# raahii/dcvgan

Measured on AMD Instinct MI355X. Metric: videos/sec per G+D step, 16x64x64 RGB+depth, higher is better.
Workload: dtype f32

## Files before the change

dcvgan_amd/csrc/conv_mfma.hip:

```cpp
#include "dcv_common.h"

#include <algorithm>
#include <cstdlib>
#include <map>
#include <mutex>
#include <string>
#include <type_traits>
#include <vector>

namespace dcv {

thread_local char g_err[512] = {0};
std::atomic<uint64_t> g_launches{0};
thread_local char g_last_kernel[160] = {0};
#define DCV_NOTE_KERNEL(...) snprintf(g_last_kernel, sizeof(g_last_kernel), __VA_ARGS__)

typedef float f32x16 __attribute__((ext_vector_type(16)));
typedef __bf16 bf16x8 __attribute__((ext_vector_type(8)));

std::atomic<int> g_precision{0};
struct BnView {
    const float* bx; const float* gamma; const float* beta; const float* mean; const float* invstd;
    int64_t bx_sn;
    int32_t bx_sc, bx_sh, cbn, act;
    float slope;
};

__device__ __forceinline__ bf16x8 pack_bf16x8(const float (&t)[8]) {
    typedef float f32x2_ __attribute__((ext_vector_type(2)));
    typedef __bf16 bf16x2_ __attribute__((ext_vector_type(2)));
    typedef uint32_t u32x4_ __attribute__((ext_vector_type(4)));
    u32x4_ w;
#pragma unroll
    for (int q = 0; q < 4; ++q) {
        const f32x2_ f = {t[2 * q], t[2 * q + 1]};
        w[q] = __builtin_bit_cast(uint32_t, __builtin_convertvector(f, bf16x2_));
    }
    return __builtin_bit_cast(bf16x8, w);
}

__device__ __forceinline__ void split3_bf16x8(const float (&t)[8], bf16x8 (&o)[3]) {
    typedef float f32x2_ __attribute__((ext_vector_type(2)));
    typedef __bf16 bf16x2_ __attribute__((ext_vector_type(2)));
    typedef uint32_t u32x4_ __attribute__((ext_vector_type(4)));
    u32x4_ h, m, l;
#pragma unroll
    for (int q = 0; q < 4; ++q) {
        const f32x2_ f = {t[2 * q], t[2 * q + 1]};
        const uint32_t hw = __builtin_bit_cast(uint32_t, __builtin_convertvector(f, bf16x2_));
        const f32x2_ r = {f[0] - __builtin_bit_cast(float, hw << 16), f[1] - __builtin_bit_cast(float, hw & 0xffff0000u)};
        const uint32_t mw = __builtin_bit_cast(uint32_t, __builtin_convertvector(r, bf16x2_));
        const f32x2_ r2 = {r[0] - __builtin_bit_cast(float, mw << 16), r[1] - __builtin_bit_cast(float, mw & 0xffff0000u)};
        h[q] = hw; m[q] = mw; l[q] = __builtin_bit_cast(uint32_t, __builtin_convertvector(r2, bf16x2_));
    }
    o[0] = __builtin_bit_cast(bf16x8, h); o[1] = __builtin_bit_cast(bf16x8, m); o[2] = __builtin_bit_cast(bf16x8, l);
}
#ifdef DCV_X6_NO_PHASES
#define X6_PHASE(IT) false
#else
#define X6_PHASE(IT) ((((IT) >> 3) & 1) != 0)
#endif
#define DCV_MFMA_X6(ACC, A3, B3)                                                              \
    {                                                                                         \
        ACC = __builtin_amdgcn_mfma_f32_32x32x16_bf16((A3)[2], (B3)[0], ACC, 0, 0, 0);        \
        ACC = __builtin_amdgcn_mfma_f32_32x32x16_bf16((A3)[0], (B3)[2], ACC, 0, 0, 0);        \
        ACC = __builtin_amdgcn_mfma_f32_32x32x16_bf16((A3)[1], (B3)[1], ACC, 0, 0, 0);        \
        ACC = __builtin_amdgcn_mfma_f32_32x32x16_bf16((A3)[1], (B3)[0], ACC, 0, 0, 0);        \
        ACC = __builtin_amdgcn_mfma_f32_32x32x16_bf16((A3)[0], (B3)[1], ACC, 0, 0, 0);        \
        ACC = __builtin_amdgcn_mfma_f32_32x32x16_bf16((A3)[0], (B3)[0], ACC, 0, 0, 0);        \
    }

#ifdef DCV_STAMP
__device__ unsigned long long g_stamp[4096][4][6];
#define STAMP(var) unsigned long long var = clock64(); __builtin_amdgcn_sched_barrier(0)
#else
#define STAMP(var) __builtin_amdgcn_sched_barrier(0)
#endif

struct KEntry {
    int32_t x_off;
    uint32_t tapsel;
    int32_t w_off;
    int32_t pad;
};

struct DimTaps {
    int32_t n;
    int32_t mul, base;
    int32_t size;
    int32_t delta[8];
};

struct GatherArgs {
    const float* x;
    float* y;
    const float* wp;
    const int32_t* koff;
    const uint32_t* ksel;
    int32_t M, OC, OCp, KIT;
    FastDiv div_sp, div_hw, div_w;
    int32_t OD, OH, OW, pad0;
    DimTaps td, th, tw;
    int64_t x_sn;
    int32_t x_sd, x_sh, x_sw, x_back;
    int64_t y_sn, y_sc, y_sd, y_sh, y_sw, y_off;
    int32_t act, accumulate;
    float slope, pad2;
    float* slab;
    int32_t kper, Mp;
    int32_t structured, s_log2p, s_stepA, s_stepD;
    int32_t s_local[16];
    uint32_t s_sel[16];
    int32_t patch, p_G, p_log2nh, p_log2tr;
    int32_t p_log2ow, p_iwp, p_ihmin, p_iwmin4;
    int32_t p_dw1, p_sc4, slab_mp, p_pad2;
    FastDiv p_gpr;
    float* stat;
    int32_t stat_ntm, stat_cls;
    const float* gate;
    float gate_slope;
    int32_t rag_m0;
};

struct GatherArgsPack {
    GatherArgs c[4];
};

__device__ __forceinline__ float apply_act(float v, int act, float slope) {
    if (act == DCV_ACT_LEAKY) return v > 0.f ? v : v * slope;
    if (act == DCV_ACT_TANH) return tanhf(v);
    return v;
}

__device__ __forceinline__ uint32_t dim_mask(const DimTaps t, int o, int shift) {
    uint32_t m = 0;
    const int p0 = o * t.mul + t.base;
#pragma unroll
    for (int u = 0; u < 8; ++u) {
        const int p = p0 + t.delta[u];
        m |= ((unsigned)p < (unsigned)t.size && u < t.n) ? (1u << (shift + u)) : 0u;
    }
    return m;
}


template <int TOC, int TM, int ACT, bool GENERIC>
__device__ __forceinline__ void store_tiles(const f32x16 (&acc)[TOC][TM], const __amdgpu_buffer_rsrc_t yrs, const uint32_t (&voff)[TM],
                                            const int ocw, const int lhi, const int OC, const uint32_t y_sc4, const int act, const float slope,
                                            const bool accumulate, const __amdgpu_buffer_rsrc_t grs, const bool gated, const float gslope) {
#pragma unroll
    for (int j = 0; j < TM; ++j)
#pragma unroll
        for (int i = 0; i < TOC; ++i)
#pragma unroll
            for (int r = 0; r < 16; ++r) {
                const int ocr = i * 32 + (r & 3) + 8 * (r >> 2);
                const uint32_t soff = (uint32_t)(ocw + ocr) * y_sc4;
                float v = acc[i][j][r];
                uint32_t vo = voff[j];
                if constexpr (GENERIC) {
                    if (ocw + ocr + 4 * lhi >= OC) vo = 0x80000000u;
                    if (accumulate) v += __builtin_bit_cast(float, __builtin_amdgcn_raw_buffer_load_b32(yrs, vo, soff, 0));
                    if (gated) v *= __builtin_bit_cast(float, __builtin_amdgcn_raw_buffer_load_b32(grs, vo, soff, 0)) > 0.f ? 1.f : gslope;
                    v = apply_act(v, act, slope);
                } else {
                    if constexpr (ACT == DCV_ACT_LEAKY) v = v > 0.f ? v : v * slope;
                    if constexpr (ACT == DCV_ACT_TANH) v = tanhf(v);
                }
                __builtin_amdgcn_raw_buffer_store_b32(__builtin_bit_cast(uint32_t, v), yrs, vo, soff, 0);
            }
}

__device__ __forceinline__ uint32_t out_voffset(const GatherArgs& a, int m, uint32_t n0, int lhi, uint32_t y_sc4) {
    if (m >= a.M) return 0x80000000u;
    const uint32_t n = fdiv((uint32_t)m, a.div_sp);
    uint32_t r0 = (uint32_t)m - n * a.div_sp.div;
    const uint32_t od = fdiv(r0, a.div_hw);
    r0 -= od * a.div_hw.div;
    const uint32_t oh = fdiv(r0, a.div_w);
    const uint32_t ow = r0 - oh * a.div_w.div;
    return 4u * (uint32_t)((int)(n - n0) * (int)a.y_sn + (int)od * (int)a.y_sd + (int)oh * (int)a.y_sh + (int)ow * (int)a.y_sw) + (uint32_t)(4 * lhi) * y_sc4;
}

template <int TOC, int TM>
__device__ __forceinline__ void gather_epilogue(const GatherArgs& a, const f32x16 (&acc)[TOC][TM], int m0, int mcol0, int l31, int lhi, int ocw, uint32_t n0) {
    const int OC = a.OC, OCp = a.OCp, act = a.act;
    const bool accumulate = a.accumulate != 0;
    const float slope = a.slope;
    const uint32_t y_sc4 = (uint32_t)a.y_sc * 4u;
    const __amdgpu_buffer_rsrc_t yrs = __builtin_amdgcn_make_buffer_rsrc(a.y + a.y_off + (int64_t)n0 * a.y_sn, 0, a.p_pad2 == 0x5701 ? 0u : 0x80000000u, 0x00020000);
    uint32_t voff[TM];
#pragma unroll
    for (int j = 0; j < TM; ++j) voff[j] = out_voffset(a, m0 + mcol0 + j * 32 + l31, n0, lhi, y_sc4);
    const bool gated = a.gate != nullptr;
    const __amdgpu_buffer_rsrc_t grs = __builtin_amdgcn_make_buffer_rsrc(const_cast<float*>(gated ? a.gate : a.y) + a.y_off + (int64_t)n0 * a.y_sn, 0, 0x80000000u, 0x00020000);
    if (OC == OCp && !accumulate && !gated) {
        if (act == DCV_ACT_NONE) store_tiles<TOC, TM, DCV_ACT_NONE, false>(acc, yrs, voff, ocw, lhi, OC, y_sc4, act, slope, false, grs, false, 0.f);
        else if (act == DCV_ACT_LEAKY) store_tiles<TOC, TM, DCV_ACT_LEAKY, false>(acc, yrs, voff, ocw, lhi, OC, y_sc4, act, slope, false, grs, false, 0.f);
        else store_tiles<TOC, TM, DCV_ACT_TANH, false>(acc, yrs, voff, ocw, lhi, OC, y_sc4, act, slope, false, grs, false, 0.f);
    } else {
        store_tiles<TOC, TM, 0, true>(acc, yrs, voff, ocw, lhi, OC, y_sc4, act, slope, accumulate, grs, gated, a.gate_slope);
    }
}

template <int TOC, int TM, int WOC, int WM, bool STRUCT>
__global__ __launch_bounds__(256, 3) void gather_gemm_kernel(const GatherArgs a) {
    constexpr int BN = 32 * TOC * WOC;
    constexpr int BM = 32 * TM * WM;
    constexpr int XPT = 16 * BM / 256;
    static_assert(WOC * WM == 4, "4 waves");
    static_assert(BM == 64 || BM == 128 || BM == 256, "BM");
    constexpr int WF4 = 16 * BN / 4;
    constexpr int WPT = (WF4 + 255) / 256;

    __shared__ __attribute__((aligned(16))) float Xs[2][16][BM];
    __shared__ __attribute__((aligned(16))) float Ws[2][16][BN];

    const int tid = threadIdx.x;
    const int lane = tid & 63;
    const int wave = __builtin_amdgcn_readfirstlane(tid >> 6);
    const int woc = wave / WM, wm = wave % WM;

    const int tiles_oc = a.OCp / BN;
    const int oc_t = blockIdx.x % tiles_oc;
    const int m_t = blockIdx.x / tiles_oc;
    const int oc0 = oc_t * BN;
    const int m0 = m_t * BM;

    const uint32_t n0 = fdiv((uint32_t)m0, a.div_sp);
    const __amdgpu_buffer_rsrc_t xrs = __builtin_amdgcn_make_buffer_rsrc(
        const_cast<float*>(a.x + (int64_t)n0 * a.x_sn), 0, 0x80000000u, 0x00020000);

    const int lm = tid % BM;
    const int ksub = __builtin_amdgcn_readfirstlane(tid / BM);
    int xbase4 = 0;
    uint32_t vmask = 0;
    {
        const int m = m0 + lm;
        if (m < a.M) {
            const uint32_t n = fdiv((uint32_t)m, a.div_sp);
            uint32_t r = (uint32_t)m - n * a.div_sp.div;
            const uint32_t od = fdiv(r, a.div_hw);
            r -= od * a.div_hw.div;
            const uint32_t oh = fdiv(r, a.div_w);
            const uint32_t ow = r - oh * a.div_w.div;
            vmask = dim_mask(a.td, (int)od, 0) | dim_mask(a.th, (int)oh, 8) | dim_mask(a.tw, (int)ow, 16);
            xbase4 = 4 * ((int)((int64_t)(n - n0) * a.x_sn) + ((int)od * a.td.mul + a.td.base) * a.x_sd +
                          ((int)oh * a.th.mul + a.th.base) * a.x_sh + ((int)ow * a.tw.mul + a.tw.base) * a.x_sw);
        }
    }

    f32x16 acc[TOC][TM];
#pragma unroll
    for (int i = 0; i < TOC; ++i)
#pragma unroll
        for (int j = 0; j < TM; ++j)
#pragma unroll
            for (int r = 0; r < 16; ++r) acc[i][j][r] = 0.f;

    float xv[XPT];
    float4 wv[WPT];

    uint32_t vloc[STRUCT ? XPT : 1];
    if constexpr (STRUCT) {
#pragma unroll
        for (int i = 0; i < XPT; ++i) {
            const int r = ksub * XPT + i;
            const uint32_t sel = a.s_sel[r];
            vloc[i] = ((vmask & sel) == sel) ? (uint32_t)(xbase4 + a.s_local[r]) : 0x80000000u;
        }
    }

    auto load_tile = [&](int it) {
        if constexpr (STRUCT) {
// ... 419 lines not shown
        if constexpr (DSTEP)
            while (nx < nst && !DCV_STEP_LIVE(DCV_IT(nx))) ++nx;
        STAMP(q0);
        asm volatile("s_waitcnt vmcnt(0)" ::: "memory");
        __syncthreads();
        STAMP(q1);
        __builtin_amdgcn_s_setprio(2);
        const int itn = DCV_IT(nx < nst ? nx : j);
        const int soffn = (itn >> a.s_log2p) * a.s_stepA + (itn & ((1 << a.s_log2p) - 1)) * a.s_stepD;
        j = nx;
        DCV_ISSUE_W(itn, buf ^ 1)
        const float* xt = Xs + buf * 16 * BM;
        const float* wt = Ws + buf * WSZ;
        if constexpr (BF == 2) {
#pragma unroll
            for (int i = 0; i < (PATCH ? NS : XPT); ++i) DCV_ISSUE_X(itn, soffn, buf ^ 1, i)
            bf16x8 a8[TOC][3], b8[TM][3];
#pragma unroll
            for (int i = 0; i < TOC; ++i)
#pragma unroll
                for (int pc = 0; pc < 3; ++pc)
                    a8[i][pc] = *reinterpret_cast<const bf16x8*>(reinterpret_cast<const char*>(wt) + 16 * ((pc * 2 + lhi) * BN + (woc * TOC + i) * 32 + l31));
            float tb[TM][8];
#pragma unroll
            for (int jj = 0; jj < TM; ++jj)
#pragma unroll
                for (int q = 0; q < 8; ++q)
                    tb[jj][q] = PATCH ? *reinterpret_cast<const float*>(reinterpret_cast<const char*>(xt) + (fbb[PATCH ? jj : 0] + koff8[PATCH ? q : 0]))
                                      : xt[(8 * lhi + q) * BM + (wm * TM + jj) * 32 + l31];
            split3_bf16x8(tb[0], b8[0]);
            if (X6_PHASE(it_cur) != x6_neg) {
                x6_neg = !x6_neg;
#pragma unroll
                for (int i = 0; i < TOC; ++i)
#pragma unroll
                    for (int jj = 0; jj < TM; ++jj)
#pragma unroll
                        for (int r = 0; r < 16; ++r) acc[i][jj][r] = -acc[i][jj][r];
            }
#pragma unroll
            for (int jj = 0; jj < TM; ++jj) {
                if (jj + 1 < TM) split3_bf16x8(tb[jj + 1 < TM ? jj + 1 : 0], b8[jj + 1 < TM ? jj + 1 : 0]);
#pragma unroll
                for (int i = 0; i < TOC; ++i) DCV_MFMA_X6(acc[i][jj], a8[i], b8[jj])
                if (jj + 1 < TM) {
#pragma unroll
                    for (int q = 0; q < 6 * TOC; ++q) {
                        __builtin_amdgcn_sched_group_barrier(0x008, 1, 0);
                        __builtin_amdgcn_sched_group_barrier(0x002, 4, 0);
                    }
                }
            }
            __builtin_amdgcn_s_setprio(0);
            continue;
        } else if constexpr (BF == 1) {
#pragma unroll
            for (int i = 0; i < (PATCH ? NS : XPT); ++i) DCV_ISSUE_X(itn, soffn, buf ^ 1, i)
            bf16x8 a8[TOC], b8[TM];
#pragma unroll
            for (int i = 0; i < TOC; ++i)
                a8[i] = *reinterpret_cast<const bf16x8*>(reinterpret_cast<const char*>(wt) + 16 * (lhi * BN + (woc * TOC + i) * 32 + l31));
#pragma unroll
            for (int jj = 0; jj < TM; ++jj) {
                float t[8];
#pragma unroll
                for (int q = 0; q < 8; ++q)
                    t[q] = PATCH ? *reinterpret_cast<const float*>(reinterpret_cast<const char*>(xt) + (fbb[PATCH ? jj : 0] + koff8[PATCH ? q : 0]))
                                 : xt[(8 * lhi + q) * BM + (wm * TM + jj) * 32 + l31];
                b8[jj] = pack_bf16x8(t);
            }
#pragma unroll
            for (int i = 0; i < TOC; ++i)
#pragma unroll
                for (int jj = 0; jj < TM; ++jj)
                    acc[i][jj] = __builtin_amdgcn_mfma_f32_32x32x16_bf16(a8[i], b8[jj], acc[i][jj], 0, 0, 0);
            __builtin_amdgcn_s_setprio(0);
            continue;
        }
        float af[2][TOC], bf[2][TM];
#pragma unroll
        for (int i = 0; i < TOC; ++i) af[0][i] = wt[lhi * BN + (woc * TOC + i) * 32 + l31];
#pragma unroll
        for (int j = 0; j < TM; ++j)
            bf[0][j] = PATCH ? *reinterpret_cast<const float*>(reinterpret_cast<const char*>(xt) + (fb[PATCH ? j : 0] + (uint32_t)koff[0]))
                             : xt[lhi * BM + (wm * TM + j) * 32 + l31];
#pragma unroll
        for (int ks = 0; ks < 8; ++ks) {
            const int cur = ks & 1, nxt = cur ^ 1;
            if (ks + 1 < 8) {
                const int k = 2 * (ks + 1) + lhi;
#pragma unroll
                for (int i = 0; i < TOC; ++i) af[nxt][i] = wt[k * BN + (woc * TOC + i) * 32 + l31];
#pragma unroll
                for (int j = 0; j < TM; ++j)
                    bf[nxt][j] = PATCH ? *reinterpret_cast<const float*>(reinterpret_cast<const char*>(xt) + (fb[PATCH ? j : 0] + (uint32_t)koff[ks + 1 < 8 ? ks + 1 : 0]))
                                       : xt[k * BM + (wm * TM + j) * 32 + l31];
            }
#pragma unroll
            for (int i = 0; i < TOC; ++i)
#pragma unroll
                for (int j = 0; j < TM; ++j)
                    acc[i][j] = __builtin_amdgcn_mfma_f32_32x32x2f32(af[cur][i], bf[cur][j], acc[i][j], 0, 0, 0);
            if constexpr (PATCH) {
                if (ks < NS) DCV_ISSUE_X(itn, soffn, buf ^ 1, ks)
            } else {
                if constexpr (XPT >= 8) {
#pragma unroll
                    for (int q = 0; q < XPT / 8; ++q) DCV_ISSUE_X(itn, soffn, buf ^ 1, ks * (XPT / 8) + q)
                } else {
                    if ((ks & 1) == 0) DCV_ISSUE_X(itn, soffn, buf ^ 1, (ks / 2) < XPT ? ks / 2 : 0)
                }
            }
            __builtin_amdgcn_sched_group_barrier(0x100, TOC + TM, 0);
            __builtin_amdgcn_sched_group_barrier(0x008, TOC * TM, 0);
            if (PATCH ? ks < NS : (XPT >= 8 || (ks & 1) == 0)) __builtin_amdgcn_sched_group_barrier(0x010, PATCH ? 1 : (XPT >= 8 ? XPT / 8 : 1), 0);
        }
        __builtin_amdgcn_s_setprio(0);
        __builtin_amdgcn_sched_barrier(0);
#ifdef DCV_STAMP
        { unsigned long long q2 = clock64(); q_wait += q1 - q0; q_loop += q2 - q1; }
#endif
    }
#ifdef DCV_STAMP
    const unsigned long long q_fw = clock64();
    __builtin_amdgcn_sched_barrier(0);
#endif
    if constexpr (BF == 2) {
        if (x6_neg) {
#pragma unroll
            for (int i = 0; i < TOC; ++i)
#pragma unroll
                for (int jj = 0; jj < TM; ++jj)
#pragma unroll
                    for (int r = 0; r < 16; ++r) acc[i][jj][r] = -acc[i][jj][r];
        }
    }
    asm volatile("s_waitcnt vmcnt(0)" ::: "memory");
#ifdef DCV_STAMP
    const unsigned long long q_epi = clock64();
#define DCV_STAMP_OUT()                                                                                      \
    if (lane == 0) {                                                                                         \
        const unsigned bid_ = blockIdx.x + gridDim.x * (blockIdx.y + gridDim.y * blockIdx.z);                \
        if (bid_ < 4096) {                                                                                   \
            unsigned long long* g = g_stamp[bid_][wave];                                                     \
            const unsigned long long q_end = clock64();                                                      \
            g[0] = q_pro - q_start; g[1] = q_wait; g[2] = q_loop; g[3] = (q_end - q_epi) | ((q_epi - q_fw) << 32); g[4] = q_end - q_start; g[5] = (unsigned long long)nst | ((q_a - q_start) << 16) | ((q_b - q_a) << 40); \
        }                                                                                                    \
    }
#else
#define DCV_STAMP_OUT()
#endif

    if (slabmode) {
        float* __restrict__ sl = a.slab + (int64_t)blockIdx.y * a.OCp * a.slab_mp;
#pragma unroll
        for (int j = 0; j < TM; ++j)
#pragma unroll
            for (int i = 0; i < TOC; ++i)
#pragma unroll
                for (int r = 0; r < 16; ++r) {
                    const int oc = oc0 + (woc * TOC + i) * 32 + (r & 3) + 8 * (r >> 2) + 4 * lhi;
                    sl[(int64_t)oc * a.slab_mp + (m0 - a.rag_m0) + (wm * TM + j) * 32 + l31] = acc[i][j][r];
                }
        DCV_STAMP_OUT()
        return;
    }
    gather_epilogue<TOC, TM>(a, acc, m0, wm * TM * 32, l31, lhi, oc0 + woc * TOC * 32, n0);
    if (a.stat) tile_bn_partials<TOC, TM, WOC, WM>(a, acc, smem, tid, lane, woc, wm, oc0, m_t);
    DCV_STAMP_OUT()
}

__global__ __launch_bounds__(256) void splitk_reduce_kernel(const GatherArgsPack pack, int S) {
    const GatherArgs& a = pack.c[blockIdx.y];
    const uint32_t Mp = (uint32_t)a.slab_mp, M = (uint32_t)a.M, q4 = Mp >> 2;
    if (q4 == 0) return;
    const uint32_t idx = blockIdx.x * 256u + threadIdx.x;
    const uint32_t oc = idx / q4, ml = (idx - oc * q4) * 4, m = ml + (uint32_t)a.rag_m0;
    if (oc >= (uint32_t)a.OC || m >= M) return;
    const float4* __restrict__ p = reinterpret_cast<const float4*>(a.slab + (int64_t)oc * Mp + ml);
    const int64_t stride = ((int64_t)a.OCp * Mp) >> 2;
    float4 v0 = {0.f, 0.f, 0.f, 0.f}, v1 = v0, v2 = v0, v3 = v0;
    int k = 0;
    for (; k + 3 < S; k += 4) {
        const float4 t0 = p[(int64_t)k * stride], t1 = p[(int64_t)(k + 1) * stride], t2 = p[(int64_t)(k + 2) * stride], t3 = p[(int64_t)(k + 3) * stride];
        v0.x += t0.x; v0.y += t0.y; v0.z += t0.z; v0.w += t0.w;
        v1.x += t1.x; v1.y += t1.y; v1.z += t1.z; v1.w += t1.w;
        v2.x += t2.x; v2.y += t2.y; v2.z += t2.z; v2.w += t2.w;
        v3.x += t3.x; v3.y += t3.y; v3.z += t3.z; v3.w += t3.w;
    }
    for (; k < S; ++k) {
        const float4 t0 = p[(int64_t)k * stride];
        v0.x += t0.x; v0.y += t0.y; v0.z += t0.z; v0.w += t0.w;
    }
    const float v[4] = {(v0.x + v1.x) + (v2.x + v3.x), (v0.y + v1.y) + (v2.y + v3.y), (v0.z + v1.z) + (v2.z + v3.z), (v0.w + v1.w) + (v2.w + v3.w)};
    const int act = a.act, accumulate = a.accumulate;
    const float slope = a.slope;
    float* __restrict__ yb = a.y + a.y_off + (int64_t)oc * a.y_sc;
#pragma unroll
    for (int e = 0; e < 4; ++e) {
        const uint32_t me = m + e;
        if (me >= M) break;
        const uint32_t n = fdiv(me, a.div_sp);
        uint32_t r0 = me - n * a.div_sp.div;
        const uint32_t od = fdiv(r0, a.div_hw);
        r0 -= od * a.div_hw.div;
        const uint32_t oh = fdiv(r0, a.div_w);
        const uint32_t ow = r0 - oh * a.div_w.div;
        float* q = yb + (int64_t)n * a.y_sn + (int64_t)od * a.y_sd + (int64_t)oh * a.y_sh + (int64_t)ow * a.y_sw;
        float x = v[e];
        if (accumulate) x += *q;
        if (a.gate) x *= a.gate[q - a.y] > 0.f ? 1.f : a.gate_slope;
        *q = apply_act(x, act, slope);
    }
}

__global__ __launch_bounds__(256) void thin_gather_kernel(const GatherArgs a) {
    __shared__ float red[3][4][64];
    const int tid = threadIdx.x, lane = tid & 63;
    const int wave = __builtin_amdgcn_readfirstlane(tid >> 6);
    const int m0 = blockIdx.x * 64;
    const uint32_t n0 = fdiv((uint32_t)m0, a.div_sp);
    const __amdgpu_buffer_rsrc_t xrs = __builtin_amdgcn_make_buffer_rsrc(
        const_cast<float*>(a.x + (int64_t)n0 * a.x_sn), 0, 0x80000000u, 0x00020000);
    const int m = m0 + lane;
    int xbase4 = 0;
    uint32_t vmask = 0;
    uint32_t n = 0, od = 0, oh = 0, ow = 0;
    if (m < a.M) {
        n = fdiv((uint32_t)m, a.div_sp);
        uint32_t r = (uint32_t)m - n * a.div_sp.div;
        od = fdiv(r, a.div_hw);
        r -= od * a.div_hw.div;
        oh = fdiv(r, a.div_w);
        ow = r - oh * a.div_w.div;
        vmask = dim_mask(a.td, (int)od, 0) | dim_mask(a.th, (int)oh, 8) | dim_mask(a.tw, (int)ow, 16);
        xbase4 = 4 * ((int)((int64_t)(n - n0) * a.x_sn) + ((int)od * a.td.mul + a.td.base) * a.x_sd +
                      ((int)oh * a.th.mul + a.th.base) * a.x_sh + ((int)ow * a.tw.mul + a.tw.base) * a.x_sw);
    }
    const int g_all = a.KIT * 4;
    const int gb0 = a.slab ? blockIdx.y * a.kper * 4 : 0;
    const int gb1 = a.slab ? min(g_all, gb0 + a.kper * 4) : g_all;
    const int gper = (gb1 - gb0 + 3) / 4;
    const int g0 = gb0 + wave * gper, g1 = min(gb1, g0 + gper);
    typedef int32_t i32x4 __attribute__((ext_vector_type(4)));
    float acc0 = 0.f, acc1 = 0.f, acc2 = 0.f, acc3 = 0.f;
    for (int g = g0; g < g1; ++g) {
        const i32x4 ko = *reinterpret_cast<const i32x4*>(a.koff + 4 * g);
        const i32x4 ks = *reinterpret_cast<const i32x4*>(a.ksel + 4 * g);
        float xv[4];
#pragma unroll
        for (int c = 0; c < 4; ++c) {
            uint32_t vo = (uint32_t)(xbase4 + ko[c]);
            vo = ((vmask & (uint32_t)ks[c]) == (uint32_t)ks[c]) ? vo : 0x80000000u;
            xv[c] = __builtin_bit_cast(float, __builtin_amdgcn_raw_buffer_load_b32(xrs, vo, 0, 0));
        }
#pragma unroll
        for (int c = 0; c < 4; ++c) {
            const float4 w = *reinterpret_cast<const float4*>(a.wp + (int64_t)(4 * g + c) * 4);
            acc0 += w.x * xv[c]; acc1 += w.y * xv[c]; acc2 += w.z * xv[c]; acc3 += w.w * xv[c];
        }
    }
    if (wave > 0) { red[wave - 1][0][lane] = acc0; red[wave - 1][1][lane] = acc1; red[wave - 1][2][lane] = acc2; red[wave - 1][3][lane] = acc3; }
    __syncthreads();
    if (wave != 0) return;
#pragma unroll
    for (int w = 0; w < 3; ++w) { acc0 += red[w][0][lane]; acc1 += red[w][1][lane]; acc2 += red[w][2][lane]; acc3 += red[w][3][lane]; }
    const float out[4] = {acc0, acc1, acc2, acc3};
    if (a.slab) {
        float* __restrict__ sl = a.slab + (int64_t)blockIdx.y * a.OCp * a.Mp;
#pragma unroll
        for (int c = 0; c < 4; ++c) sl[(int64_t)c * a.Mp + m] = out[c];
        return;
    }
    if (m >= a.M) return;
    float* __restrict__ yb = a.y + a.y_off + (int64_t)n * a.y_sn + (int64_t)od * a.y_sd + (int64_t)oh * a.y_sh + (int64_t)ow * a.y_sw;
#pragma unroll
    for (int c = 0; c < 4; ++c)
        if (c < a.OC) {
            float v = out[c];
            float* q = yb + (int64_t)c * a.y_sc;
            if (a.accumulate) v += *q;
            *q = apply_act(v, a.act, a.slope);
        }
}

template <int T, int NOC>
__global__ __launch_bounds__(256) void thin_struct_kernel(const GatherArgs a, int RC, int rc_per_split) {
    __shared__ float red[3][4][64];
    const int tid = threadIdx.x, lane = tid & 63;
    const int wave = __builtin_amdgcn_readfirstlane(tid >> 6);
    const int m0 = blockIdx.x * 64;
    const uint32_t n0 = fdiv((uint32_t)m0, a.div_sp);
    const __amdgpu_buffer_rsrc_t xrs = __builtin_amdgcn_make_buffer_rsrc(
        const_cast<float*>(a.x + (int64_t)n0 * a.x_sn), 0, 0x80000000u, 0x00020000);
    const int m = m0 + lane;
    int xbase4 = 0;
    uint32_t vmask = 0;
    uint32_t n = 0, od = 0, oh = 0, ow = 0;
    if (m < a.M) {
        n = fdiv((uint32_t)m, a.div_sp);
        uint32_t r = (uint32_t)m - n * a.div_sp.div;
        od = fdiv(r, a.div_hw);
        r -= od * a.div_hw.div;
        oh = fdiv(r, a.div_w);
        ow = r - oh * a.div_w.div;
        vmask = dim_mask(a.td, (int)od, 0) | dim_mask(a.th, (int)oh, 8) | dim_mask(a.tw, (int)ow, 16);
        xbase4 = 4 * ((int)((int64_t)(n - n0) * a.x_sn) + ((int)od * a.td.mul + a.td.base) * a.x_sd +
                      ((int)oh * a.th.mul + a.th.base) * a.x_sh + ((int)ow * a.tw.mul + a.tw.base) * a.x_sw);
    }
    uint32_t vloc[T];
#pragma unroll
    for (int t = 0; t < T; ++t) {
        const uint32_t sel = a.s_sel[t];
        vloc[t] = ((vmask & sel) == sel) ? (uint32_t)(xbase4 + a.s_local[t]) : 0x80000000u;
    }
    const int cb0 = a.slab ? blockIdx.y * rc_per_split : 0;
// ... 1646 lines not shown
        const float* __restrict__ wc = wq + (int64_t)c * (ND * 16);
#pragma unroll
        for (int kd = 0; kd < ND; ++kd)
#pragma unroll
            for (int aa = 0; aa < 2; ++aa)
#pragma unroll
                for (int bb = 0; bb < 2; ++bb) acc[kd][aa][bb] += xv * wc[kd * 16 + aa * 8 + bb * 2];
    }
#pragma unroll
    for (int kd = 0; kd < ND; ++kd)
#pragma unroll
        for (int aa = 0; aa < 2; ++aa)
#pragma unroll
            for (int bb = 0; bb < 2; ++bb) S[q][lane][kd * 4 + aa * 2 + bb] = acc[kd][aa][bb];
    __syncthreads();
    const int t_pj = tid >> 6, t_kd = (tid >> 4) & 3, oh = (tid >> 2) & 3, ow = tid & 3;
    const int t_pidx = (int)blockIdx.x * 4 + t_pj;
    if (t_kd >= ND || t_pidx >= NP) return;
    float sum = 0.f;
#pragma unroll
    for (int kh = 0; kh < 4; ++kh) {
        const int hh = 2 * oh - 1 + kh;
        if (hh < 0 || hh > 7) continue;
#pragma unroll
        for (int kw = 0; kw < 4; ++kw) {
            const int ww = 2 * ow - 1 + kw;
            if (ww < 0 || ww > 7) continue;
            sum += S[(hh & 1) * 2 + (ww & 1)][t_pj * 16 + (hh >> 1) * 4 + (ww >> 1)][t_kd * 4 + (kh >> 1) * 2 + (kw >> 1)];
        }
    }
    a.part[(((int64_t)blockIdx.y * NP + t_pidx) * ND + t_kd) * 16 + oh * 4 + ow] = sum;
}

template <int ND>
__global__ __launch_bounds__(256) void head_fwd_combine_kernel(const HeadArgs a) {
    const int64_t i = (int64_t)blockIdx.x * 256 + threadIdx.x;
    const int64_t tot = (int64_t)a.N * a.OD * 16;
    if (i >= tot) return;
    const int pos = (int)(i & 15);
    const int64_t r = i >> 4;
    const int n = (int)(r / a.OD), od = (int)(r - (int64_t)n * a.OD);
    const int NP = a.N * a.D;
    float sum = 0.f;
    for (int cs = 0; cs < a.CS; ++cs)
#pragma unroll
        for (int kd = 0; kd < ND; ++kd) sum += a.part[(((int64_t)cs * NP + (int64_t)n * a.D + od + kd) * ND + kd) * 16 + pos];
    a.out[(int64_t)n * a.y_sn + (int64_t)od * a.y_sd + pos] = apply_act(sum, a.act, a.slope);
}

template <int ND>
__global__ __launch_bounds__(256) void head_dgrad_kernel(const HeadArgs a) {
    DCV_HEAD_LANES()
    const int NP = a.N * a.D;
    const int pidx = (int)blockIdx.x * 4 + pj;
    if (pidx >= NP) return;
    const int n = pidx / a.D, d = pidx - n * a.D;
    float g[ND][2][2];
#pragma unroll
    for (int kd = 0; kd < ND; ++kd)
#pragma unroll
        for (int aa = 0; aa < 2; ++aa)
#pragma unroll
            for (int bb = 0; bb < 2; ++bb) {
                const int od = d - kd, oh = i_ + ph - aa, ow = j_ + pw - bb;
                const bool ok = od >= 0 && od < a.OD && (unsigned)oh < 4u && (unsigned)ow < 4u;
                g[kd][aa][bb] = ok ? a.dy[(int64_t)n * a.y_sn + (int64_t)od * a.y_sd + oh * 4 + ow] : 0.f;
            }
    float* __restrict__ op = a.out + (int64_t)n * a.x_sn + (int64_t)d * a.x_sd + h * 8 + w_;
    const float* __restrict__ wq = a.w + (1 - ph) * 4 + (1 - pw);
    const int c0 = (int)blockIdx.y * a.cper, c1 = min(a.C, c0 + a.cper);
#pragma unroll 4
    for (int c = c0; c < c1; ++c) {
        const float* __restrict__ wc = wq + (int64_t)c * (ND * 16);
        float v = 0.f;
#pragma unroll
        for (int kd = 0; kd < ND; ++kd)
#pragma unroll
            for (int aa = 0; aa < 2; ++aa)
#pragma unroll
                for (int bb = 0; bb < 2; ++bb) v += g[kd][aa][bb] * wc[kd * 16 + aa * 8 + bb * 2];
        float* o = op + (int64_t)c * a.x_sc;
        *o = a.accumulate ? *o + v : v;
    }
}

template <int ND, int CG>
__global__ __launch_bounds__(256) void head_wgrad_kernel(const HeadArgs a) {
    DCV_HEAD_LANES()
    const int NP = a.N * a.D, c0 = (int)blockIdx.x * CG;
    const int ngroups = (NP + 3) / 4, gper = (ngroups + (int)gridDim.y - 1) / (int)gridDim.y;
    const int g0 = (int)blockIdx.y * gper, g1 = min(ngroups, g0 + gper);
    float acc[CG][ND * 4];
#pragma unroll
    for (int cc = 0; cc < CG; ++cc)
#pragma unroll
        for (int e = 0; e < ND * 4; ++e) acc[cc][e] = 0.f;
    int pos[4];
    bool pok[4];
#pragma unroll
    for (int ab = 0; ab < 4; ++ab) {
        const int oh = i_ + ph - (ab >> 1), ow = j_ + pw - (ab & 1);
        pok[ab] = (unsigned)oh < 4u && (unsigned)ow < 4u;
        pos[ab] = pok[ab] ? oh * 4 + ow : 0;
    }
    const float* __restrict__ xc = a.x + (int64_t)c0 * a.x_sc + h * 8 + w_;
    for (int gi = g0; gi < g1; ++gi) {
        const int pidx = gi * 4 + pj;
        const bool valid = pidx < NP;
        const int n = valid ? pidx / a.D : 0, d = valid ? pidx - n * a.D : 0;
        float gv[ND * 4];
#pragma unroll
        for (int kd = 0; kd < ND; ++kd) {
            const int od = d - kd;
            const bool dok = valid && od >= 0 && od < a.OD;
            const float* __restrict__ gp = a.dy + (int64_t)n * a.y_sn + (int64_t)(dok ? od : 0) * a.y_sd;
#pragma unroll
            for (int ab = 0; ab < 4; ++ab) gv[kd * 4 + ab] = (dok && pok[ab]) ? gp[pos[ab]] : 0.f;
        }
        const float* __restrict__ xp = xc + (int64_t)n * a.x_sn + (int64_t)d * a.x_sd;
#pragma unroll
        for (int cc = 0; cc < CG; ++cc) {
            const float xv = (valid && c0 + cc < a.C) ? xp[(int64_t)cc * a.x_sc] : 0.f;
#pragma unroll
            for (int e = 0; e < ND * 4; ++e) acc[cc][e] += xv * gv[e];
        }
    }
    float* __restrict__ out = a.part + ((int64_t)blockIdx.y * a.C) * (ND * 16);
#pragma unroll
    for (int cc = 0; cc < CG; ++cc)
#pragma unroll
        for (int e = 0; e < ND * 4; ++e) {
            float v = acc[cc][e];
#pragma unroll
            for (int off = 32; off > 0; off >>= 1) v += __shfl_xor(v, off, 64);
            if (lane == 0 && c0 + cc < a.C)
                out[(int64_t)(c0 + cc) * (ND * 16) + (e >> 2) * 16 + ((1 - ph) + 2 * ((e >> 1) & 1)) * 4 + (1 - pw) + 2 * (e & 1)] = v;
        }
}
#undef DCV_HEAD_LANES

struct DevTable {
    KEntry* dev = nullptr;
    int32_t* koff = nullptr;
    uint32_t* ksel = nullptr;
    int rows = 0;
};

static std::mutex g_plan_mu;
static std::map<std::string, DevTable> g_tables;

struct Toggles {
    bool no_lds_dma, no_dstep, no_patch, no_row64, no_widen, no_widen_mfma, no_thinj_wgrad, no_wgrad_dma, no_wgrad_dma64, no_quad, no_thin_wgrad;
    int half_m;
    bool no_ragged, no_wgrad_d16, no_head_kernels, no_stem3d_wgrad, wgrad_x6;
    int stem3d_stages;
#ifdef DCV_DEBUG_TIMING
    bool debug_nostore;
#endif
    Toggles() {
        auto on = [](const char* n) { return getenv(n) != nullptr; };
        no_lds_dma = on("DCV_NO_LDS_DMA"); no_dstep = on("DCV_NO_DSTEP"); no_patch = on("DCV_NO_PATCH"); no_row64 = on("DCV_NO_ROW64");
        no_widen = on("DCV_NO_WIDEN"); no_widen_mfma = on("DCV_NO_WIDEN_MFMA"); no_thinj_wgrad = on("DCV_NO_THINJ_WGRAD"); no_wgrad_dma = on("DCV_NO_WGRAD_DMA"); no_wgrad_dma64 = on("DCV_NO_WGRAD_DMA64"); no_quad = on("DCV_NO_QUAD"); no_thin_wgrad = on("DCV_NO_THIN_WGRAD");
        half_m = getenv("DCV_HALF_M") ? atoi(getenv("DCV_HALF_M")) : -1;
        no_ragged = on("DCV_NO_RAGGED");
        no_wgrad_d16 = on("DCV_NO_WGRAD_D16");
        no_head_kernels = on("DCV_NO_HEAD_KERNELS"); no_stem3d_wgrad = on("DCV_NO_STEM3D_WGRAD"); wgrad_x6 = on("DCV_WGRAD_X6");
        stem3d_stages = getenv("DCV_STEM3D_STAGES") ? atoi(getenv("DCV_STEM3D_STAGES")) : 0;
#ifdef DCV_DEBUG_TIMING
        debug_nostore = on("DCV_DEBUG_NOSTORE");
#endif
    }
};
static const Toggles& toggles() {
    static const Toggles t;
    return t;
}

struct HeadBnRequest {
    int mode;
    const float* bx; dcv_dims5 bxd; float* bdx; dcv_dims5 bdxd;
    const float* gamma; const float* beta; const float* mean; const float* invstd;
    const float* cst; float* partial; size_t partial_bytes;
    int cbn; float slope;
};

struct CallOpts {
    int precision = 0;
    int wgrad_acc = 0;
    const BnView* bnview = nullptr;
    const HeadBnRequest* headbn = nullptr;
};
static int call_opts(const dcv_conv_geom* g, CallOpts* o, const char* tag) {
    if (g && (g->mfma < 0 || g->mfma > 3))
        return fail(DCV_EINVAL, "%s: dcv_conv_geom.mfma must be 0 (process default), 1 (fp32), 2 (bf16 products) or 3 (fp32 on the bf16 pipe)", tag);
    o->precision = g && g->mfma > 0 ? g->mfma - 1 : g_precision.load(std::memory_order_relaxed);
    return DCV_OK;
}

static std::string device_prefix() {
    int dev = 0;
    (void)hipGetDevice(&dev);
    char b[16];
    const int n = snprintf(b, sizeof(b), "d%d|", dev);
    return std::string(b, n);
}

template <class Build>
static int get_table(const std::string& key, Build build, DevTable* out) {
    std::lock_guard<std::mutex> lk(g_plan_mu);
    auto it = g_tables.find(key);
    if (it != g_tables.end()) {
        *out = it->second;
        return DCV_OK;
    }
    const std::vector<KEntry> host = build();
    DevTable t;
    t.rows = (int)host.size();
    DCV_HIP_CHECK(hipMalloc((void**)&t.dev, host.size() * sizeof(KEntry)));
    DCV_HIP_CHECK(hipMemcpy(t.dev, host.data(), host.size() * sizeof(KEntry), hipMemcpyHostToDevice));
    {
        std::vector<int32_t> off(host.size());
        std::vector<uint32_t> sel(host.size());
        for (size_t i = 0; i < host.size(); ++i) {
            off[i] = host[i].x_off * 4;
            sel[i] = host[i].tapsel;
        }
        DCV_HIP_CHECK(hipMalloc((void**)&t.koff, host.size() * sizeof(int32_t)));
        DCV_HIP_CHECK(hipMalloc((void**)&t.ksel, host.size() * sizeof(uint32_t)));
        DCV_HIP_CHECK(hipMemcpy(t.koff, off.data(), off.size() * sizeof(int32_t), hipMemcpyHostToDevice));
        DCV_HIP_CHECK(hipMemcpy(t.ksel, sel.data(), sel.size() * sizeof(uint32_t), hipMemcpyHostToDevice));
    }
    g_tables[key] = t;
    *out = t;
    return DCV_OK;
}

static void tap_offsets(const DimTaps& t, int64_t stride, int64_t* lo, int64_t* hi) {
    *lo = *hi = (int64_t)t.delta[0] * stride;
    for (int u = 1; u < t.n; ++u) {
        *lo = std::min(*lo, (int64_t)t.delta[u] * stride);
        *hi = std::max(*hi, (int64_t)t.delta[u] * stride);
    }
}

static bool tap_span(const DimTaps& t, int* dmin) {
    int lo = t.delta[0], hi = t.delta[0];
    for (int u = 1; u < t.n; ++u) { lo = std::min(lo, t.delta[u]); hi = std::max(hi, t.delta[u]); }
    *dmin = lo;
    return hi - lo + 1 == t.n;
}

struct GatherClass {
    int o_ext[3];
    int out_mul[3], out_off[3];
    DimTaps taps[3];
    std::vector<int> tap_k[3];
};
static bool live(const GatherClass& c) {
    return c.taps[0].n * c.taps[1].n * c.taps[2].n > 0 && c.o_ext[0] > 0 && c.o_ext[1] > 0 && c.o_ext[2] > 0;
}

struct TileCfg {
    int bn, bm;
};

static TileCfg pick_gather_tile(int OC) {
    if (OC <= 4) return {4, 64};
    if (OC > 64 && OC % 128 != 0 && OC % 64 == 0 && OC <= 448) return {64, 256};
    if (OC > 64) return {128, 128};
    if (OC > 32) return {64, 256};
    return {32, 256};
}

template <int TOC, int TM, int WOC, int WM>
static void launch_gather(const GatherArgs& a, dim3 grid, hipStream_t s) {
    if (a.structured) hipLaunchKernelGGL((gather_gemm_kernel<TOC, TM, WOC, WM, true>), grid, dim3(256), 0, s, a);
    else hipLaunchKernelGGL((gather_gemm_kernel<TOC, TM, WOC, WM, false>), grid, dim3(256), 0, s, a);
}

struct RagPlan { int t1, k; };
static RagPlan rag_plan(int64_t W, int grp) {
    RagPlan p{0, 1};
    if (toggles().no_ragged || grp <= 0 || W < 1024 + 16) return p;
    const int64_t F = W / 1024;
    if (F > 2) return p;
    const int64_t t1 = (F * 1024 / grp) & ~7ll;
    const int64_t E = W - t1 * grp;
    constexpr int target = 512;
    if (t1 <= 0 || E <= 0 || E >= target) return p;
    p.t1 = (int)t1;
    p.k = (int)((target + E - 1) / E);
    if (p.k > 16) p.k = 16;
    return p;
}

static int gather_splits(int blocks, int KIT, bool thin) {
    const int min_steps = thin ? 16 : 8;
    if (blocks >= 384 || KIT < 2 * min_steps) return 1;
    int ks = (768 + blocks - 1) / blocks;
    const int maxks = KIT / min_steps;
    if (ks > maxks) ks = maxks;
    if (ks > 64) ks = 64;
    return ks < 1 ? 1 : ks;
}

static int flush_packs(const float* w, const PackArgs& packs, int n, int kmax, int OC, int OCp, int64_t ws_o, hipStream_t stream) {
    const int64_t tot = (int64_t)kmax * OCp;
    hipLaunchKernelGGL(pack_weights_kernel, dim3((unsigned)((tot + 255) / 256), (unsigned)n), dim3(256), 0, stream, w, packs, OC, OCp, ws_o);
    DCV_LAUNCH_CHECK();
    return DCV_OK;
}

static int flush_pending(GatherArgsPack& pend, int n, dim3 grid, const TileCfg& tc, int KS, int OC, int bfm, hipStream_t stream) {
    for (int i = n; i < 4; ++i) pend.c[i] = pend.c[0];
    {
        const unsigned tiles_oc = (unsigned)(pend.c[0].OCp / tc.bn);
        const unsigned ntm = (grid.x + tiles_oc - 1) / tiles_oc;
        grid.x = (ntm + 7) / 8 * 8 * tiles_oc * (unsigned)n;
        grid.z = 1;
        pend.c[0].pad0 = n;
    }
    const bool ds = pend.c[0].structured == 2, pt = pend.c[0].patch != 0;
#define DCV_LAUNCH_DMA1(A, B, C_, D, BF_)                                                                                     \
    {                                                                                                                         \
        if (ds && pt) hipLaunchKernelGGL((gather_gemm_dma_kernel<A, B, C_, D, true, true, BF_>), grid, dim3(256), 0, stream, pend); \
        else if (ds) hipLaunchKernelGGL((gather_gemm_dma_kernel<A, B, C_, D, true, false, BF_>), grid, dim3(256), 0, stream, pend); \
        else if (pt) hipLaunchKernelGGL((gather_gemm_dma_kernel<A, B, C_, D, false, true, BF_>), grid, dim3(256), 0, stream, pend); \
        else hipLaunchKernelGGL((gather_gemm_dma_kernel<A, B, C_, D, false, false, BF_>), grid, dim3(256), 0, stream, pend);        \
    }
#define DCV_LAUNCH_DMA(A, B, C_, D)                                                                                           \
    {                                                                                                                         \
        if (bfm == 2) DCV_LAUNCH_DMA1(A, B, C_, D, 2) else if (bfm == 1) DCV_LAUNCH_DMA1(A, B, C_, D, 1) else DCV_LAUNCH_DMA1(A, B, C_, D, 0) \
    }
    if (tc.bn == 128 && tc.bm == 64) DCV_LAUNCH_DMA(2, 1, 2, 2)
    else if (tc.bn == 64 && tc.bm == 128) DCV_LAUNCH_DMA(2, 1, 1, 4)
    else if (tc.bn == 128) DCV_LAUNCH_DMA(2, 2, 2, 2)
    else if (tc.bn == 64) DCV_LAUNCH_DMA(2, 2, 1, 4)
    else DCV_LAUNCH_DMA(1, 2, 1, 4)
#undef DCV_LAUNCH_DMA
#undef DCV_LAUNCH_DMA1
    DCV_NOTE_KERNEL("gather_gemm_dma_kernel<%s, %s, %s, %s> (%d x %d tile, %d class%s in one launch%s%s)",
                    tc.bn == 128 ? (tc.bm == 64 ? "2, 1, 2, 2" : "2, 2, 2, 2") : tc.bn == 64 ? (tc.bm == 128 ? "2, 1, 1, 4" : "2, 2, 1, 4") : "1, 2, 1, 4",
                    ds ? "true" : "false", pt ? "true" : "false", bfm == 2 ? "2" : bfm ? "1" : "0", tc.bn, tc.bm, n, n == 1 ? "" : "es", KS > 1 ? (pend.c[0].rag_m0 > 0 ? ", ragged split-K" : ", split-K") : "",
                    bfm == 2 ? ", f32x6: fp32 on the bf16 pipe" : bfm ? ", bf16 products" : "");
    DCV_LAUNCH_CHECK();
    if (KS > 1) {
        int64_t tot = 0;
        for (int i = 0; i < n; ++i) tot = std::max<int64_t>(tot, (int64_t)OC * (pend.c[i].slab_mp / 4));
        if (tot == 0) return DCV_OK;
        hipLaunchKernelGGL(splitk_reduce_kernel, dim3((unsigned)((tot + 255) / 256), (unsigned)n), dim3(256), 0, stream, pend, KS);
        DCV_LAUNCH_CHECK();
    }
    return DCV_OK;
}

static int structured_walk(const GatherClass& c, const dcv_dims5& xd, int RC, bool dstep, bool thin) {
    if (thin) return 0;
    if (dstep) return 2;
    const int nd = c.taps[0].n, THW = c.taps[1].n * c.taps[2].n, T = nd * THW;
    const int64_t sc4 = xd.sc * 4;
    if (T > 0 && 16 % T == 0 && RC % (16 / T) == 0 && sc4 * (16 / T) < (1ll << 30)) return 1;
    if (THW == 16 && (nd == 2 || nd == 4 || nd == 8) && c.taps[0].mul == 1 && c.taps[0].base == 0 &&
        c.taps[0].delta[nd - 1] == nd - 1 && c.o_ext[0] + nd - 1 <= c.taps[0].size && sc4 < (1ll << 30)) return 3;
    return 0;
}

static inline size_t pack_elem_bytes(int precision) { return precision == 2 ? 6 : sizeof(float); }

struct GatherOp {
    const float* x = nullptr; float* y = nullptr; const float* w = nullptr;
    dcv_dims5 xd{}, yd{};
    int RC = 0, OC = 0, KH = 1, KW = 1;
    int64_t ws_o = 0, ws_r = 0;
    std::vector<GatherClass> classes;
    int act = DCV_ACT_NONE, accumulate = 0;
    float slope = 0.f;
    bool stats = false;
    float* stat = nullptr; size_t stat_bytes = 0;
    const dcv_wpack* pack = nullptr;
    const float* gate = nullptr; float gate_slope = 0.f;
    const char* tag = "";
};

enum class GK { Dma, Rows, RowsBn, HeadBn, WidenMfma, WidenRows, ThinStruct, ThinGather, Gemm };
struct ClassPlan {
    GatherArgs a;
    GK kind;
    dim3 grid;
    size_t ci;
    bool dstep;
    bool stat;
    int T, KS2, fmt;
    int rows_kind, rows_iw0;
    int groups;
    size_t wp_off, slab_off;
};
struct GatherPlan {
    TileCfg tc{};
    int OCp = 0;
    std::vector<ClassPlan> cls;
    size_t ws_need = 0, pack_need = 0, stat_need = 0;
    bool stat_memset = false;
    int stat_parts = 0;
};

static int plan_gather(const GatherOp& op, const CallOpts& o, GatherPlan* P) {
    const Toggles& tg = toggles();
    const dcv_dims5 &xd = op.xd, &yd = op.yd;
    const int RC = op.RC, OC = op.OC;
    const char* tag = op.tag;
    TileCfg tc = pick_gather_tile(OC);
    int nlive = 0, stat_ntm = 0, ntm_min = INT32_MAX;
    auto workgroups = [&](int bm) {
        int64_t W = 0;
        for (const GatherClass& c : op.classes)
            if (live(c)) W += ((OC + tc.bn - 1) / tc.bn) * (((int64_t)yd.n * c.o_ext[0] * c.o_ext[1] * c.o_ext[2] + bm - 1) / bm);
        return W;
    };
    for (const GatherClass& c : op.classes) nlive += live(c);
    if (tc.bn >= 64) {
        const int64_t W = workgroups(tc.bm);
        const double rounds = (double)W / 1024.0, frac = rounds - (double)(int64_t)rounds;
        bool half = (rounds > 0.4 && rounds < 1.0) || (rounds >= 1.0 && rounds < 3.0 && frac > 0.15 && frac < 0.55);
        if (tg.half_m >= 0) half = tg.half_m != 0;
        if (half && rounds >= 1.0 && tg.half_m < 0 && !tg.no_lds_dma && nlive > 0 && W / nlive >= 384 &&
            rag_plan(W, ((OC + tc.bn - 1) / tc.bn) * nlive).k > 1) half = false;
        if (half) tc.bm /= 2;
    }
    RagPlan rag{0, 1};
    if (tc.bn >= 64 && !tg.no_lds_dma) {
        rag = rag_plan(workgroups(tc.bm), ((OC + tc.bn - 1) / tc.bn) * nlive);
        if (op.stats && (int64_t)OC * yd.n * yd.d * yd.h * yd.w * 4 > (160ll << 20)) rag.k = 1;
    }
    if (op.gate && tc.bn == 4) return fail(DCV_EUNSUPPORTED, "%s: the gated epilogue is not built into the thin (OC <= 4) kernels", tag);
    if (op.gate)
        for (const GatherClass& c : op.classes)
            if (c.taps[0].n * c.taps[1].n * c.taps[2].n == 0 && c.o_ext[0] > 0 && c.o_ext[1] > 0 && c.o_ext[2] > 0)
                return fail(DCV_EUNSUPPORTED, "%s: gated epilogue with a tap-less position class", tag);
    const int OCp = (OC + tc.bn - 1) / tc.bn * tc.bn;
    P->tc = tc; P->OCp = OCp; P->cls.clear(); P->pack_need = 0;
    for (const GatherClass& c : op.classes) {
        if (!live(c)) continue;
        const int ntm = (int)(((int64_t)yd.n * c.o_ext[0] * c.o_ext[1] * c.o_ext[2] + tc.bm - 1) / tc.bm);
        stat_ntm = std::max(stat_ntm, ntm);
        ntm_min = std::min(ntm_min, ntm);
    }
    P->stat_need = (size_t)nlive * stat_ntm * OCp * 2 * sizeof(float);
    bool stat_ok = op.stats && op.act == DCV_ACT_NONE && !op.accumulate && tc.bn != 4 && P->stat_need > 0 && P->stat_need <= op.stat_bytes;
    P->stat_memset = stat_ok && ntm_min != stat_ntm;
    const bool own_pack = op.pack && op.pack->buf;
    size_t pk_off = 0, ws_off = 0;
    int stat_ci = 0;
    for (size_t ci = 0; ci < op.classes.size(); ++ci) {
        const GatherClass& c = op.classes[ci];
        if (!live(c)) continue;
        ClassPlan cp{};
        memset(&cp.a, 0, sizeof(cp.a));
        cp.ci = ci;
        const int T = c.taps[0].n * c.taps[1].n * c.taps[2].n;
        const int64_t K = (int64_t)RC * T;
        const int KIT = (int)((K + 15) / 16);
        const int64_t M64 = (int64_t)yd.n * c.o_ext[0] * c.o_ext[1] * c.o_ext[2];
        if (M64 >= (1ll << 31)) return fail(DCV_EUNSUPPORTED, "%s: too many positions", tag);
        bool dstep = false;
        {
            const DimTaps& t0 = c.taps[0];
            const int nd = t0.n;
            if (tc.bn != 4 && (nd == 2 || nd == 4 || nd == 8) && c.taps[1].n * c.taps[2].n == 4 && RC % 4 == 0 && t0.mul == 1 &&
                xd.sc * 16 < (1ll << 30) && xd.sd * 4 * nd < (1ll << 30) && !tg.no_lds_dma && !tg.no_dstep) {
                bool consecutive = true;
                for (int u = 0; u < nd; ++u) consecutive = consecutive && t0.delta[u] == -u;
                const bool padded = t0.base - (nd - 1) < 0 || c.o_ext[0] - 1 + t0.base >= t0.size;
                dstep = consecutive && padded;
            }
        }
        {
            int64_t lo = std::min<int64_t>(0, (int64_t)(RC - 1) * xd.sc), hi = std::max<int64_t>(0, (int64_t)(RC - 1) * xd.sc);
            const int64_t strides[3] = {xd.sd, xd.sh, xd.sw};
            for (int d = 0; d < 3; ++d) {
                int64_t l, h;
                tap_offsets(c.taps[d], strides[d], &l, &h);
                lo += l;
                hi += h;
            }
            if (hi > INT32_MAX / 4 || lo < INT32_MIN / 4) return fail(DCV_EUNSUPPORTED, "%s: tensor too large for 32-bit offsets", tag);
        }
        const int Mp = (int)((M64 + tc.bm - 1) / tc.bm * tc.bm);
        const int blocks = (OCp / tc.bn) * (Mp / tc.bm);
        int KS = gather_splits(tc.bn != 4 && !dstep ? blocks * (int)op.classes.size() : blocks, KIT, tc.bn == 4);
        if (o.bnview) KS = 1;
        const int walk = structured_walk(c, xd, RC, dstep, tc.bn == 4);
        const bool dma = walk != 0 && !tg.no_lds_dma;
        int rag_m0 = 0;
        if (KS == 1 && rag.k > 1 && dma && KIT / rag.k >= 8) {
            KS = rag.k;
            rag_m0 = (int)std::min<int64_t>((int64_t)rag.t1 * tc.bm, Mp);
        } else if (rag.k > 1 && KS == 1) {
            rag.k = 1;
        }
// ... 1251 lines not shown
```

Before: 655.8.

## Fold split-K reduction into GEMM launch via per-tile atomic tickets

Split-K partial tiles are now written in a tile-contiguous layout, and each block increments a per-tile atomic ticket. The last block to arrive sums all partials and runs the normal epilogue itself. This removes the separate splitk_reduce_kernel launch and its extra pass over the slab. In exchange it adds release/acquire fences and a serial reduction done by one block per tile, and it keeps a persistent ticket buffer per stream that must return to zero after every launch.

Measured after the change: 655.2. About the same (-0.1%).

```diff
diff --git a/dcvgan_amd/csrc/conv_mfma.hip b/dcvgan_amd/csrc/conv_mfma.hip
--- a/dcvgan_amd/csrc/conv_mfma.hip
+++ b/dcvgan_amd/csrc/conv_mfma.hip
@@ -120,6 +120,7 @@
     const float* gate;
     float gate_slope;
     int32_t rag_m0;
+    uint32_t* tickets;
 };
 
 struct GatherArgsPack {
@@ -845,16 +846,92 @@
 #endif
 
     if (slabmode) {
-        float* __restrict__ sl = a.slab + (int64_t)blockIdx.y * a.OCp * a.slab_mp;
+        uint32_t* const tickets = a.tickets;
+        if (tickets == nullptr) {
+            float* __restrict__ sl = a.slab + (int64_t)blockIdx.y * a.OCp * a.slab_mp;
+#pragma unroll
+            for (int j = 0; j < TM; ++j)
+#pragma unroll
+                for (int i = 0; i < TOC; ++i)
+#pragma unroll
+                    for (int r = 0; r < 16; ++r) {
+                        const int oc = oc0 + (woc * TOC + i) * 32 + (r & 3) + 8 * (r >> 2) + 4 * lhi;
+                        sl[(int64_t)oc * a.slab_mp + (m0 - a.rag_m0) + (wm * TM + j) * 32 + l31] = acc[i][j][r];
+                    }
+            DCV_STAMP_OUT()
+            return;
+        }
+        const uint32_t S = gridDim.y;
+        const uint32_t part_bytes = (uint32_t)a.OCp * (uint32_t)a.slab_mp * 4u;
+        char* const tile0 = reinterpret_cast<char*>(a.slab + ((int64_t)((m0 - a.rag_m0) / BM) * (a.OCp / BN) + oc_t) * (BN * BM));
+        const uint32_t svo = (uint32_t)((wave * (TOC * TM * 4)) * 64 + lane) * 16u;
+        {
+            char* const mine = tile0 + blockIdx.y * part_bytes;
+#pragma unroll
+            for (int j = 0; j < TM; ++j)
+#pragma unroll
+                for (int i = 0; i < TOC; ++i)
+#pragma unroll
+                    for (int q = 0; q < 4; ++q)
+                        *reinterpret_cast<float4*>(mine + ((j * TOC + i) * 4 + q) * 1024 + svo) =
+                            float4{acc[i][j][4 * q], acc[i][j][4 * q + 1], acc[i][j][4 * q + 2], acc[i][j][4 * q + 3]};
+        }
+        asm volatile("s_waitcnt vmcnt(0)" ::: "memory");
+        __syncthreads();
+        if (tid == 0) {
+            __builtin_amdgcn_fence(__ATOMIC_RELEASE, "agent");
+            asm volatile("s_waitcnt vmcnt(0)" ::: "memory");
+            const uint32_t ticket = __hip_atomic_fetch_add(tickets + blockIdx.x, 1u, __ATOMIC_RELAXED, __HIP_MEMORY_SCOPE_AGENT);
+            const bool last = ticket == S - 1;
+            if (last) {
+                __hip_atomic_store(tickets + blockIdx.x, 0u, __ATOMIC_RELAXED, __HIP_MEMORY_SCOPE_AGENT);
+                __builtin_amdgcn_fence(__ATOMIC_ACQUIRE, "agent");
+                asm volatile("s_waitcnt vmcnt(0)" ::: "memory");
+            }
+            smem[0] = last ? 1.f : 0.f;
+        }
+        __syncthreads();
+        if (smem[0] == 0.f) {
+            DCV_STAMP_OUT()
+            return;
+        }
+        auto part = [&](uint32_t so) { return *reinterpret_cast<const float4*>((tile0 + so) + svo); };
+#define DCV_ADD4(V, T) V.x += T.x; V.y += T.y; V.z += T.z; V.w += T.w;
 #pragma unroll
         for (int j = 0; j < TM; ++j)
 #pragma unroll
-            for (int i = 0; i < TOC; ++i)
-#pragma unroll
-                for (int r = 0; r < 16; ++r) {
-                    const int oc = oc0 + (woc * TOC + i) * 32 + (r & 3) + 8 * (r >> 2) + 4 * lhi;
-                    sl[(int64_t)oc * a.slab_mp + (m0 - a.rag_m0) + (wm * TM + j) * 32 + l31] = acc[i][j][r];
+            for (int i = 0; i < TOC; ++i) {
+                f32x16 sum[1][1];
+#pragma unroll
+                for (int q = 0; q < 4; ++q) {
+                    uint32_t so = (uint32_t)(((j * TOC + i) * 4 + q) * 1024);
+                    float4 v0 = {0.f, 0.f, 0.f, 0.f}, v1 = v0, v2 = v0, v3 = v0;
+                    uint32_t k = 0;
+                    if constexpr (TOC * TM < 4)
+#pragma unroll 1
+                    for (; k + 7 < S; k += 8, so += 8 * part_bytes) {
+                        const float4 t0 = part(so), t1 = part(so + part_bytes), t2 = part(so + 2 * part_bytes), t3 = part(so + 3 * part_bytes);
+                        const float4 t4 = part(so + 4 * part_bytes), t5 = part(so + 5 * part_bytes), t6 = part(so + 6 * part_bytes), t7 = part(so + 7 * part_bytes);
+                        DCV_ADD4(v0, t0) DCV_ADD4(v1, t1) DCV_ADD4(v2, t2) DCV_ADD4(v3, t3)
+                        DCV_ADD4(v0, t4) DCV_ADD4(v1, t5) DCV_ADD4(v2, t6) DCV_ADD4(v3, t7)
+                    }
+#pragma unroll 1
+                    for (; k + 3 < S; k += 4, so += 4 * part_bytes) {
+                        const float4 t0 = part(so), t1 = part(so + part_bytes), t2 = part(so + 2 * part_bytes), t3 = part(so + 3 * part_bytes);
+                        DCV_ADD4(v0, t0) DCV_ADD4(v1, t1) DCV_ADD4(v2, t2) DCV_ADD4(v3, t3)
+                    }
+#pragma unroll 1
+                    for (; k < S; ++k, so += part_bytes) {
+                        const float4 t0 = part(so);
+                        DCV_ADD4(v0, t0)
+                    }
+                    float r0 = (v0.x + v1.x) + (v2.x + v3.x), r1 = (v0.y + v1.y) + (v2.y + v3.y), r2 = (v0.z + v1.z) + (v2.z + v3.z), r3 = (v0.w + v1.w) + (v2.w + v3.w);
+                    asm volatile("" : "+v"(r0), "+v"(r1), "+v"(r2), "+v"(r3));
+                    sum[0][0][4 * q] = r0; sum[0][0][4 * q + 1] = r1; sum[0][0][4 * q + 2] = r2; sum[0][0][4 * q + 3] = r3;
                 }
+                gather_epilogue<1, 1>(a, sum, m0, (wm * TM + j) * 32, l31, lhi, oc0 + (woc * TOC + i) * 32, n0);
+            }
+#undef DCV_ADD4
         DCV_STAMP_OUT()
         return;
     }
@@ -2807,7 +2884,7 @@
 struct Toggles {
     bool no_lds_dma, no_dstep, no_patch, no_row64, no_widen, no_widen_mfma, no_thinj_wgrad, no_wgrad_dma, no_wgrad_dma64, no_quad, no_thin_wgrad;
     int half_m;
-    bool no_ragged, no_wgrad_d16, no_head_kernels, no_stem3d_wgrad, wgrad_x6;
+    bool no_ragged, no_wgrad_d16, no_head_kernels, no_stem3d_wgrad, wgrad_x6, no_splitk_inlaunch;
     int stem3d_stages;
 #ifdef DCV_DEBUG_TIMING
     bool debug_nostore;
@@ -2821,6 +2898,7 @@
         no_wgrad_d16 = on("DCV_NO_WGRAD_D16");
         no_head_kernels = on("DCV_NO_HEAD_KERNELS"); no_stem3d_wgrad = on("DCV_NO_STEM3D_WGRAD"); wgrad_x6 = on("DCV_WGRAD_X6");
         stem3d_stages = getenv("DCV_STEM3D_STAGES") ? atoi(getenv("DCV_STEM3D_STAGES")) : 0;
+        no_splitk_inlaunch = on("DCV_NO_SPLITK_INLAUNCH");
 #ifdef DCV_DEBUG_TIMING
         debug_nostore = on("DCV_DEBUG_NOSTORE");
 #endif
@@ -2966,6 +3044,23 @@
     return DCV_OK;
 }
 
+constexpr unsigned kTicketWords = 16384;
+constexpr int kInlaunchMaxParts = 16;
+static std::mutex g_ticket_mu;
+static std::map<std::pair<int, hipStream_t>, uint32_t*> g_tickets;
+static uint32_t* ticket_pool(hipStream_t stream) {
+    int dev = 0;
+    if (hipGetDevice(&dev) != hipSuccess) return nullptr;
+    std::lock_guard<std::mutex> lk(g_ticket_mu);
+    auto it = g_tickets.find({dev, stream});
+    if (it != g_tickets.end()) return it->second;
+    uint32_t* p = nullptr;
+    if (hipMalloc(reinterpret_cast<void**>(&p), kTicketWords * sizeof(uint32_t)) != hipSuccess) { (void)hipGetLastError(); return nullptr; }
+    if (hipMemsetAsync(p, 0, kTicketWords * sizeof(uint32_t), stream) != hipSuccess) { (void)hipGetLastError(); (void)hipFree(p); return nullptr; }
+    g_tickets[{dev, stream}] = p;
+    return p;
+}
+
 static int flush_pending(GatherArgsPack& pend, int n, dim3 grid, const TileCfg& tc, int KS, int OC, int bfm, hipStream_t stream) {
     for (int i = n; i < 4; ++i) pend.c[i] = pend.c[0];
     {
@@ -2975,6 +3070,13 @@
         grid.z = 1;
         pend.c[0].pad0 = n;
     }
+    uint32_t* tickets = nullptr;
+    if (KS > 1 && KS <= kInlaunchMaxParts && grid.x <= kTicketWords && !toggles().no_splitk_inlaunch) {
+        int64_t bytes = 0;
+        for (int i = 0; i < n; ++i) bytes = std::max<int64_t>(bytes, (int64_t)KS * pend.c[i].OCp * pend.c[i].slab_mp * 4);
+        if (bytes < (1ll << 31)) tickets = ticket_pool(stream);
+    }
+    for (int i = 0; i < 4; ++i) pend.c[i].tickets = tickets;
     const bool ds = pend.c[0].structured == 2, pt = pend.c[0].patch != 0;
 #define DCV_LAUNCH_DMA1(A, B, C_, D, BF_)                                                                                     \
     {                                                                                                                         \
@@ -2999,7 +3101,7 @@
                     ds ? "true" : "false", pt ? "true" : "false", bfm == 2 ? "2" : bfm ? "1" : "0", tc.bn, tc.bm, n, n == 1 ? "" : "es", KS > 1 ? (pend.c[0].rag_m0 > 0 ? ", ragged split-K" : ", split-K") : "",
                     bfm == 2 ? ", f32x6: fp32 on the bf16 pipe" : bfm ? ", bf16 products" : "");
     DCV_LAUNCH_CHECK();
-    if (KS > 1) {
+    if (KS > 1 && tickets == nullptr) {
         int64_t tot = 0;
         for (int i = 0; i < n; ++i) tot = std::max<int64_t>(tot, (int64_t)OC * (pend.c[i].slab_mp / 4));
         if (tot == 0) return DCV_OK;
```
